# TheNeodev/RVC-MAKER

Measured on AMD Instinct MI355X. Metric: audio-seconds/sec/GPU (xRT) end-to-end VC, 48k v2; 1/2/4/8 GPU scaling, higher is better.
Workload: dtype f32-equivalent (split-fp16 3-pass MFMA for the generator's convs -- scale from the producer's published |max| -- and ResBlock pairs, split-bf16 6-pass MFMA elsewhere; f32 accumulate; RMVPE f64 with its GRU recurrence f32); 1 GPU; VC.pipeline 48k v2, ContentVec-768, rmvpe f0, one 30 s clip per GPU per step, no index, protect 0.33, clip stream (clip k+1 f0/features under clip k synthesizer); model=RVC v2 48k (NSF-HiFiGAN) + ContentVec + rmvpe, global_batch=1, seq_len=480000, parallelism=utterance-sharded x1

## Files before the change

### include/rvc_amd.h

```cpp
#ifndef RVC_AMD_H
#define RVC_AMD_H

#include <stdint.h>

#ifdef __cplusplus
extern "C" {
#endif

typedef struct ihipStream_t* rvc_stream_t;

enum { RVC_OK = 0, RVC_EINVAL = -22, RVC_EHIP = -5 };

enum {
    RVC_ACT_NONE = 0,
    RVC_ACT_LRELU = 1,
    RVC_ACT_RELU = 2,
    RVC_ACT_TANH = 3,
    RVC_ACT_GELU = 4,
    RVC_ACT_SIGMOID = 5,
    RVC_ACT_LOGCLAMP = 6,
};

const char* rvc_last_error(void);
int rvc_version(void);
// ... 20 lines not shown
    int toff[16];
    const void* wx;
    int wx_nmf, wx_passes;
    const unsigned* amax_in;
    unsigned* amax_out;
    const float* src_x;
    const float* src_w;
    const float* src_b;
    int src_K, src_stride, src_pad, _pad1;
    int64_t src_len, src_bstride;
} rvc_conv1d_args;

int64_t rvc_conv1d_workspace_bytes(const rvc_conv1d_args* a);
int rvc_conv1d_engine(const rvc_conv1d_args* a);
int rvc_conv1d_tile(const rvc_conv1d_args* a);
int rvc_conv1d(const rvc_conv1d_args* a, void* ws, int64_t ws_bytes, rvc_stream_t stream);
void rvc_conv1d_set_probe_event(void* hip_event);
int rvc_conv1d_set_stamps(void* buf, int64_t bytes);
int rvc_resblock_set_stamps(void* buf, int64_t bytes);
int rvc_resblock_set_ylds(int on);
int rvc_resblock_set_wide64(int on);
int rvc_conv1d_set_tile_epi(int on);
int rvc_conv1d_set_swz(int on);
int rvc_conv1d_set_f16_fast(int on);
int rvc_conv1d_set_splitk_target(int target);
int rvc_stream_create_cu_mask(const uint32_t* mask, int nwords, rvc_stream_t* out);
int rvc_stream_destroy(rvc_stream_t stream);
int64_t rvc_conv1d_x6_bytes(int64_t nphase, int64_t Ci, int K, int64_t Co);
int rvc_conv1d_pack_x6(const float* w_km, int64_t nphase, int64_t Ci, int K, int64_t Co, void* out, int* nmf_out,
                       rvc_stream_t stream);
int64_t rvc_conv1d_f16_bytes(int64_t nphase, int64_t Ci, int K, int64_t Co);
int rvc_conv1d_pack_f16(const float* w_km, int64_t nphase, int64_t Ci, int K, int64_t Co, void* out, int* nmf_out,
                        rvc_stream_t stream);

typedef struct rvc_resblock_args {
    const float* x;
    float* y;
    const void* w1x;
    const float* b1;
    const void* w2x;
    const float* b2;
    int64_t C, L;
    int K, dil, nmf1, nmf2, passes, accumulate;
    float slope;
    int B;
} rvc_resblock_args;
// ... 456 lines not shown
```

### rvc-maker_amd/csrc/conv1d.hip

```cpp
#include "rvc_common.h"
#include "x6_common.h"
#include <stdlib.h>
#include <type_traits>
#include <algorithm>

namespace {

constexpr int KCH = 32;
constexpr int NB_MAX = 16;

struct ConvParams {
    const float* x;
    const float* w;
    const float* bias;
    const float* bias2;
    const float* res;
    float* y;
    float* ws;
    int64_t B, Ci, Co, Lin, Lout, ncols;
    int64_t x_bstride, y_bstride, res_bstride, w_bstride;
    int K, stride, dil, pad, groups;
    int nphase, ostride, ooffset;
    int in_act, out_act, accumulate;
    float in_scale, in_slope, out_slope, out_scale;
    int span, span_s, rows_max;
    float inv_span;
    int mtiles_per_group, ksplit, chunks_per_split, avec;
    int ntoff, wrap;
    int toff[16];
    const uint4* wx;
    int wx_nmf, wx_nch, wx_passes;
    int rot;
    int xcd;
    int dbg;
    int tile_epi;
    const unsigned* amax_in;
    int f16_fast;
    unsigned* amax_out;
    int stagger;
    int stagger_blocks;
    int swz;
    int gx6;
#if RVC_CONV_STAMPS
    unsigned long long* stamps;
    int64_t stamp_blocks;
#endif
};

static thread_local int g_f16_fast = -1;
static thread_local int g_swz = -1;

__device__ __forceinline__ int tap_off(const ConvParams& p, int t) { return p.ntoff ? p.toff[t] : t * p.dil; }

__device__ __forceinline__ int out_pos(const ConvParams& p, int64_t n, int phase) {
    if (n >= p.ncols) return -1;
    const int t = (int)n * p.ostride + p.ooffset + phase;
    if (t < 0 || t >= (int)p.Lout) return -1;
    if (p.wrap) {
        const int row = t / p.wrap, col = t - row * p.wrap;
        if (col == 0 || col == p.wrap - 1 || row == 0 || row == (int)p.Lout / p.wrap - 1) return -(t + 2);
    }
    return t;
}

__device__ __forceinline__ float epilogue_store(const ConvParams& p, float acc, int b, int64_t m, int t) {
    const bool ok = t >= 0;
    const int64_t o = m * p.Lout + (ok ? t : 0);
    float v = acc;
    if (p.bias) v += p.bias[m];
    if (p.bias2) v += p.bias2[m];
    v = act_apply(v, p.out_act, p.out_slope) * p.out_scale;
    if (p.res) v += p.res[b * p.res_bstride + o];
    float* yb = p.y + b * p.y_bstride;
// ... 648 lines not shown
    }
    if (p.amax_out && !part) amax_publish(p.amax_out + (int64_t)b * RVC_AMAX_SHARDS, amx);
}

template <int FM, int FN, int WM, int WN, int X6_NI, int NP, bool F16, bool SA = false, int LF = 0>
__global__ __launch_bounds__(64 * (WM * WN + 4), (x6_min_blocks<FM, FN, WM * WN, NP>())) void conv_x6_kernel(ConvParams p) {
    static_assert(WM * WN == 4 || WM * WN == 8, "4 or 8 compute waves");
    constexpr int NCW = WM * WN;
    static_assert(NP == 6 || NP == 3 || NP == 1, "6, 3 or 1 passes");
    static_assert(!F16 || NP == 3, "split-fp16: 3 passes");
    static_assert(!SA || (NP == 6 && !F16), "split accumulators: 6-pass split-bf16");
    static_assert(LF == 0 || (F16 && WM * WN == 8), "fast-only loaders: split-fp16 on 8 compute waves");
    constexpr int NPL = NP == 6 ? 3 : (NP == 3 ? 2 : 1);
    constexpr int BM = 16 * FM * WM;
    constexpr int BN = 16 * FN * WN;
    extern __shared__ uint4 xs[];
    const int tid = threadIdx.x, lane = tid & 63;
    const int wave = __builtin_amdgcn_readfirstlane(tid >> 6);
    int bx = blockIdx.x, by = blockIdx.y, bz = blockIdx.z;
    if (p.xcd) {
        const int nx = gridDim.x, ny = gridDim.y;
        const int nwg = nx * ny * (int)gridDim.z;
        const int orig = bx + nx * (by + ny * bz);
        const int q = nwg >> 3, r = nwg & 7, xc = orig & 7;
        const int t = (xc < r ? xc * (q + 1) : r * (q + 1) + (xc - r) * q) + (orig >> 3);
        bx = t % nx;
        by = (t / nx) % ny;
        bz = t / (nx * ny);
    }
    int zb = bz;
    const int split = zb % p.ksplit;
    zb /= p.ksplit;
    const int phase = zb % p.nphase;
    const int b = zb / p.nphase;
    const int grp = p.gx6 ? phase : 0;
    const int ophase = p.gx6 ? 0 : phase;
    const int Cog = (int)p.Co;
    const int Cig = (int)p.Ci;
    const int m0g = by * BM;
    const int64_t n0 = (int64_t)bx * BN;
    const int K = p.K, span = p.span;
    const int nch = p.wx_nch, nmf = p.wx_nmf;
    const int ch_beg = split * p.chunks_per_split;
    const int ch_end = min(nch, ch_beg + p.chunks_per_split);
    const int nck = ch_end - ch_beg;
    const int bufsz = NPL * span * 4;
    float* tmax = reinterpret_cast<float*>(xs + 2 * bufsz);
    float* etab = tmax + 4;
    const int rseed = p.rot ? (bx >> 3) : 0;
    const int rt = rseed % K, rc = (rseed / K) % max(nck, 1);
    auto pchunk = [&](int i) __attribute__((always_inline)) {
// ... 567 lines not shown
        }
    }
    float yo[SRC_M];
#pragma unroll
    for (int mi = 0; mi < SRC_M; ++mi) yo[mi] = yb[(int64_t)(m0 + (mi < nm ? mi : 0)) * p.Lout];
    float amx = 0.f;
#pragma unroll
    for (int mi = 0; mi < SRC_M; ++mi) {
        if (mi < nm) {
            const int m = m0 + mi;
            const float v = (acc[mi] + (p.b ? p.b[m] : 0.f)) + yo[mi];
            if (ok) {
                yb[(int64_t)m * p.Lout] = v;
                amx = fmaxf(amx, fabsf(v));
            }
        }
    }
    if (p.amax_out) amax_publish_block(p.amax_out + (int64_t)b * RVC_AMAX_SHARDS, amx);
}

struct Cfg {
    int FM, FN, WM, WN;
    bool x6;
};

template <int FM, int FN, int WM, int WN>
hipError_t launch(const ConvParams& p, dim3 grid, size_t lds, hipStream_t s) {
    hipLaunchKernelGGL((conv1d_mfma_kernel<FM, FN, WM, WN>), grid, dim3(256), lds, s, p);
    return hipGetLastError();
}

template <int FM, int FN, int WM, int WN, int NP, bool F16 = false, bool SA = false, int LF = 0>
void launch_x6_np(const ConvParams& p, dim3 grid, size_t lds, hipStream_t s) {
    const dim3 blk(64 * (WM * WN + 4));
    if (4 * p.span <= 256 * 3)
        hipLaunchKernelGGL((conv_x6_kernel<FM, FN, WM, WN, 3, NP, F16, SA, LF>), grid, blk, lds, s, p);
    else hipLaunchKernelGGL((conv_x6_kernel<FM, FN, WM, WN, 6, NP, F16, SA, LF>), grid, blk, lds, s, p);
}

int x6_f16_fast_form(const ConvParams& p) {
    if (!p.amax_in || !p.f16_fast || (p.Ci & 31) != 0 || p.in_scale != 1.f) return 0;
    return p.in_act == RVC_ACT_LRELU ? 1 : (p.in_act == RVC_ACT_NONE ? 2 : 0);
}

constexpr bool x6_sa_tile(int FM, int FN, int WM, int WN) {
    return (WM * WN == 8 && FN == 4) || (WM * WN == 4 && FM <= 2 && FN == 2) || (WM == 2 && WN == 4);
// ... 39 lines not shown
    for (int i = 0; i < 16; ++i) p.toff[i] = a->ntoff ? a->toff[i] : 0;
    p.wx = nullptr;
    p.wx_nmf = p.wx_nch = 0;
    p.wx_passes = a->wx_passes == 0 ? 6 : a->wx_passes;
    static const int dbg = getenv("RVC_CONV_DEBUG") ? atoi(getenv("RVC_CONV_DEBUG")) : 0;
    p.dbg = dbg;
    p.tile_epi = 0;
    p.amax_in = a->amax_in;
    p.amax_out = a->amax_out;
    static const int f16fast = getenv("RVC_X6_F16FAST") ? atoi(getenv("RVC_X6_F16FAST")) : 1;
    p.f16_fast = g_f16_fast >= 0 ? g_f16_fast : f16fast;
    p.stagger = 0;
    p.stagger_blocks = 0;
    static const int swz_env = getenv("RVC_X6_SWZ") ? atoi(getenv("RVC_X6_SWZ")) : 1;
    p.swz = g_swz >= 0 ? g_swz : swz_env;
    p.gx6 = 0;
#if RVC_CONV_STAMPS
    p.stamps = g_stamps;
    p.stamp_blocks = g_stamp_blocks;
#endif
    static const int rot = getenv("RVC_X6_ROT") ? atoi(getenv("RVC_X6_ROT")) : 0;
    p.rot = rot;
    static const int xcd = getenv("RVC_X6_XCD") ? atoi(getenv("RVC_X6_XCD")) : 1;
    p.xcd = xcd;
}

int num_cus() {
    static const int n = [] {
        int dev = 0, cus = 0;
        if (hipGetDevice(&dev) != hipSuccess ||
            hipDeviceGetAttribute(&cus, hipDeviceAttributeMultiprocessorCount, dev) != hipSuccess || cus <= 0)
            cus = 256;
        return cus;
    }();
    return n;
}

static thread_local int g_splitk_target = -1;
static thread_local int g_tile_epi = -1;

void split_k(ConvParams& p, int64_t tiles, int nch, int per_cu = 2) {
    static const int env_target = getenv("RVC_SPLITK_TILES") ? atoi(getenv("RVC_SPLITK_TILES")) : 256;
    static const int occ_aware = getenv("RVC_X6_SPLIT_OCC") ? atoi(getenv("RVC_X6_SPLIT_OCC")) : 1;
    int target = g_splitk_target >= 0 ? g_splitk_target : env_target;
    if (occ_aware && per_cu == 1 && g_splitk_target < 0) target /= 2;
    int ks = 1;
    if (tiles < target && nch >= 4) {
// ... 38 lines not shown

int plan(const rvc_conv1d_args* a, ConvParams& p, Cfg& cfg, dim3& grid, size_t& lds) {
    RVC_CHECK_ARG(a && a->x && a->w && a->y, "conv1d: null pointer");
    RVC_CHECK_ARG(a->B > 0 && a->Ci > 0 && a->Co > 0 && a->K > 0 && a->Lin > 0 && a->Lout > 0,
                  "conv1d: bad sizes B=%lld Ci=%lld Co=%lld K=%d Lin=%lld Lout=%lld", (long long)a->B,
                  (long long)a->Ci, (long long)a->Co, a->K, (long long)a->Lin, (long long)a->Lout);
    RVC_CHECK_ARG(a->groups >= 1 && a->Ci % a->groups == 0 && a->Co % a->groups == 0, "conv1d: bad groups");
    RVC_CHECK_ARG(a->stride >= 1 && a->dil >= 1 && a->nphase >= 1 && a->ostride >= 1, "conv1d: bad stride/dil");
    RVC_CHECK_ARG(a->Co * a->Lout < (1ll << 31) && a->Ci * a->Lin < (1ll << 31) && a->Lin + a->pad < (1ll << 30),
                  "conv1d: per-batch tensor exceeds 2^31 elements (use the batch dimension)");
    const int64_t Cog = a->Co / a->groups;
    const int64_t Cig = a->Ci / a->groups;
    const int64_t ncols = a->ncols > 0 ? a->ncols : a->Lout;
    fill_common(a, p);
    RVC_CHECK_ARG(!a->src_x || (a->src_w && a->src_K > 0 && a->src_K <= 4096 && a->src_stride > 0 && a->src_pad >= 0 &&
                                a->src_len > 0 && a->src_bstride >= 0 && !a->wrap),
                  "conv1d: bad fused source conv (src_K=%d src_stride=%d src_pad=%d src_len=%lld)", a->src_K,
                  a->src_stride, a->src_pad, (long long)a->src_len);
    RVC_CHECK_ARG(!a->src_x || ((int64_t)255 * a->src_stride + 17 * a->src_K) * 4 <= 64 * 1024,
                  "conv1d: source conv span too large (stride %d, K %d)", a->src_stride, a->src_K);
    if (a->ntoff) {
        RVC_CHECK_ARG(a->ntoff == a->K && a->K <= 16, "conv1d: toff needs ntoff == K <= 16");
        for (int i = 0; i < a->K; ++i) RVC_CHECK_ARG(a->toff[i] >= 0, "conv1d: negative tap offset");
    }

    if (x6_eligible(a)) {
        cfg.x6 = true;
        static const int w8 = getenv("RVC_X6_W8") ? atoi(getenv("RVC_X6_W8")) : 1;
        const int np = a->wx_passes == 0 || a->wx_passes == RVC_ARITH_FP32_SA ? 6 : a->wx_passes;
        static const int bn256 = getenv("RVC_X6_BN256") ? atoi(getenv("RVC_X6_BN256")) : 1;
        auto round_eff = [](int64_t t) {
            const int64_t n = num_cus();
            return (double)t / (double)(((t + n - 1) / n) * n);
        };
        const int64_t rows128 = (Cog + 127) / 128, nb = a->B * a->nphase;
        const bool fills256 = round_eff(rows128 * ((ncols + 255) / 256) * nb) >=
                              round_eff(rows128 * ((ncols + 127) / 128) * nb) - 0.05;
        if (Cog > 64 && w8 && bn256 && a->stride == 1 && 255 + max_tap_off(a) + 1 <= 64 * X6_NI_MAX - 2 &&
            Cog % 16 == 0 && a->Lout < (1ll << 26) && ncols < (1ll << 26) &&
            (bn256 == 2 || np == RVC_ARITH_F16X3) && (fills256 || bn256 == 3))
            cfg = {2, 8, 4, 2, true};
        else if (Cog > 64 && w8) cfg = {2, 4, 4, 2, true};
        else if (Cog > 64) cfg = {4, 4, 2, 2, true};
        else if (Cog > 32 && w8 && np >= 3) cfg = {2, 2, 2, 4, true};
        else if (Cog > 32) cfg = {2, 4, 2, 2, true};
        else if (Cog > 16) cfg = {2, 2, 1, 4, true};
// ... 1 lines not shown
        RVC_CHECK_ARG(a->wx_passes != RVC_ARITH_FP32_SA || x6_sa_tile(cfg.FM, cfg.FN, cfg.WM, cfg.WN),
                      "conv1d: RVC_ARITH_FP32_SA has no split-accumulator kernel for the %dx%d tile on %d waves "
                      "(engine switches changed?)", 16 * cfg.FM * cfg.WM, 16 * cfg.FN * cfg.WN, cfg.WM * cfg.WN);
        const int BM = 16 * cfg.FM * cfg.WM, BN = 16 * cfg.FN * cfg.WN;
        p.span = (BN - 1) * a->stride + max_tap_off(a) + 1;
        p.span_s = p.span;
        p.rows_max = 0;
        p.inv_span = 1.0f / (float)p.span;
        p.avec = 0;
        p.wx = (const uint4*)a->wx;
        p.wx_nmf = a->wx_nmf;
        p.wx_nch = (int)((Cig + 31) / 32);
        p.mtiles_per_group = (int)((Cog + BM - 1) / BM);
        const int64_t tiles = (int64_t)p.mtiles_per_group * ((ncols + BN - 1) / BN) * a->B * a->nphase * a->groups;
        split_k(p, tiles, p.wx_nch, cfg.WM * cfg.WN == 8 ? 1 : 2);
        if (a->groups > 1) {
            p.gx6 = 1;
            p.nphase = a->groups;
            p.Ci = Cig;
            p.Co = Cog;
            p.chunks_per_split = p.wx_nch;
            p.ksplit = 1;
        }
        lds = (size_t)2 * (p.wx_passes == 6 || p.wx_passes == RVC_ARITH_FP32_SA ? 3 : (p.wx_passes == 1 ? 1 : 2)) *
              p.span * 64 + 16;
        static const int tepi_env = getenv("RVC_X6_TILE_EPI") ? atoi(getenv("RVC_X6_TILE_EPI")) : 0;
        const int tepi = g_tile_epi >= 0 ? g_tile_epi : tepi_env;
        const size_t tile_bytes = (size_t)BM * (BN + 4) * 4;
        const bool plain = a->nphase == 1 && a->ostride == 1 && a->ooffset == 0 && !a->wrap && !(p.dbg & 1) &&
                           BN <= 128;
        p.tile_epi = !(tepi && plain && a->groups == 1) ? 0
                     : tile_bytes <= lds ? 1 : (cfg.WM % 2 == 0 && tile_bytes / 2 <= lds) ? 2 : 0;
        lds += (size_t)3 * BM * 4;
        grid = dim3(cdiv(ncols, BN), (unsigned)p.mtiles_per_group, (unsigned)(a->B * p.nphase * p.ksplit));
        RVC_CHECK_ARG(grid.y < 65536 && grid.z < 65536, "conv1d: grid too large");
        static const int stagger = getenv("RVC_X6_STAGGER") ? atoi(getenv("RVC_X6_STAGGER")) : 0;
        static const int stagger_rounds = getenv("RVC_X6_STAGGER_ROUNDS") ? atoi(getenv("RVC_X6_STAGGER_ROUNDS")) : 2;
        const int64_t nblk = (int64_t)grid.x * grid.y * grid.z;
        if (stagger > 0 && nblk >= stagger_rounds * (int64_t)num_cus()) {
            p.stagger = stagger;
            p.stagger_blocks = num_cus();
        }
        return RVC_OK;
    }

    if (Cog % 48 == 0 && Cog % 64 != 0) cfg = {3, 1, 1, 4, false};
// ... 139 lines not shown
    RVC_CHECK_ARG(w_km && out && nmf_out && nphase > 0 && Ci > 0 && K > 0 && Co > 0, "pack_f16: bad args");
    const int nch = (int)((Ci + 31) / 32), nmf = (int)x6_nmf(Co);
    const int64_t total = nphase * K * nch * nmf * 3 * 64;
    float* rs = reinterpret_cast<float*>(reinterpret_cast<uint4*>(out) + total);
    hipStream_t s = (hipStream_t)stream;
    const int64_t nrow = nphase * Ci * K;
    RVC_HIP(hipMemsetAsync(rs, 0, (size_t)nmf * 16 * 4, s));
    hipLaunchKernelGGL(rowscale_f16_kernel, dim3(cdiv(Co, 64), (unsigned)std::min<int64_t>(64, cdiv(nrow, 64))),
                       dim3(256), 0, s, w_km, nrow, (int)Co, reinterpret_cast<unsigned*>(rs));
    hipLaunchKernelGGL(rowscale_fin_kernel, dim3(cdiv(nmf * 16, 256)), dim3(256), 0, s, rs, nmf * 16);
    hipLaunchKernelGGL(pack_f16_kernel, dim3(cdiv(total, 256)), dim3(256), 0, s, w_km, total, (int)Ci, K, (int)Co, nch,
                       nmf, (const float*)rs, (uint4*)out);
    RVC_HIP(hipGetLastError());
    *nmf_out = nmf;
    return RVC_OK;
}

extern "C" int rvc_conv1d_engine(const rvc_conv1d_args* a) {
    ConvParams p;
    Cfg cfg;
    dim3 grid;
    size_t lds;
    if (plan(a, p, cfg, grid, lds) != RVC_OK) return -1;
    return cfg.x6 ? 1 : 0;
}

extern "C" int rvc_conv1d_tile(const rvc_conv1d_args* a) {
    ConvParams p;
    Cfg cfg;
    dim3 grid;
    size_t lds;
    if (plan(a, p, cfg, grid, lds) != RVC_OK) return -1;
    return (16 * cfg.FM * cfg.WM) << 16 | (16 * cfg.FN * cfg.WN);
}

extern "C" int64_t rvc_conv1d_workspace_bytes(const rvc_conv1d_args* a) {
    ConvParams p;
    Cfg cfg;
    dim3 grid;
    size_t lds;
    if (plan(a, p, cfg, grid, lds) != RVC_OK) return -1;
    if (p.ksplit <= 1) return 0;
    return (int64_t)p.ksplit * p.B * p.nphase * p.Co * p.ncols * 4;
}

extern "C" int rvc_conv1d_set_splitk_target(int target) {
    const int prev = g_splitk_target;
    g_splitk_target = target < 0 ? -1 : target;
    return prev;
}

static thread_local hipEvent_t g_probe_event = nullptr;

extern "C" void rvc_conv1d_set_probe_event(void* hip_event) { g_probe_event = (hipEvent_t)hip_event; }

extern "C" int rvc_conv1d_set_f16_fast(int on) {
    g_f16_fast = on < 0 ? -1 : (on ? 1 : 0);
    return RVC_OK;
}

extern "C" int rvc_conv1d_set_swz(int on) {
    g_swz = on < 0 ? -1 : (on ? 1 : 0);
    return RVC_OK;
}

extern "C" int rvc_conv1d_set_tile_epi(int on) {
    g_tile_epi = on < 0 ? -1 : (on ? 1 : 0);
    return RVC_OK;
}

extern "C" int rvc_conv1d_set_stamps(void* buf, int64_t bytes) {
#if RVC_CONV_STAMPS
    g_stamps = (unsigned long long*)buf;
    g_stamp_blocks = buf ? bytes / (8 * X6_STAMP_W) : 0;
    return 0;
#else
    (void)buf;
    (void)bytes;
    return -1;
#endif
}

extern "C" int rvc_conv1d(const rvc_conv1d_args* a, void* ws, int64_t ws_bytes, rvc_stream_t stream) {
    ConvParams p;
    Cfg cfg;
    dim3 grid;
    size_t lds;
    int rc = plan(a, p, cfg, grid, lds);
    if (rc != RVC_OK) return rc;
    if (p.ksplit > 1) {
        const int64_t need = (int64_t)p.ksplit * p.B * p.nphase * p.Co * p.ncols * 4;
        RVC_CHECK_ARG(ws && ws_bytes >= need, "conv1d: split-K needs %lld B of workspace (got %lld)",
                      (long long)need, (long long)ws_bytes);
        p.ws = (float*)ws;
    }
    hipStream_t s = (hipStream_t)stream;
    if (a->src_x) p.amax_out = nullptr;
    hipError_t e;
    if (cfg.x6) {
        if (cfg.WM == 4 && cfg.FN == 8) e = launch_x6<2, 8, 4, 2>(p, grid, lds, s);
        else if (cfg.WM == 4) e = launch_x6<2, 4, 4, 2>(p, grid, lds, s);
        else if (cfg.WM == 2 && cfg.WN == 4) e = launch_x6<2, 2, 2, 4>(p, grid, lds, s);
        else if (cfg.FM == 4) e = launch_x6<4, 4, 2, 2>(p, grid, lds, s);
        else if (cfg.WM == 2) e = launch_x6<2, 4, 2, 2>(p, grid, lds, s);
        else if (cfg.FM == 2) e = launch_x6<2, 2, 1, 4>(p, grid, lds, s);
        else e = launch_x6<1, 2, 1, 4>(p, grid, lds, s);
    } else if (cfg.FM == 3) e = launch<3, 1, 1, 4>(p, grid, lds, s);
    else if (cfg.FM == 1 && cfg.FN == 4) e = launch<1, 4, 1, 4>(p, grid, lds, s);
    else if (cfg.FM == 1) e = launch<1, 2, 1, 4>(p, grid, lds, s);
    else if (cfg.WM == 1 && cfg.FN == 4) e = launch<2, 4, 1, 4>(p, grid, lds, s);
    else if (cfg.WM == 1) e = launch<2, 2, 1, 4>(p, grid, lds, s);
    else if (cfg.FM == 4 && cfg.FN == 4) e = launch<4, 4, 2, 2>(p, grid, lds, s);
    else if (cfg.FM == 4) e = launch<4, 2, 2, 2>(p, grid, lds, s);
    else if (cfg.FN == 4) e = launch<2, 4, 2, 2>(p, grid, lds, s);
    else e = launch<2, 2, 2, 2>(p, grid, lds, s);
    RVC_HIP(e);
    if (g_probe_event) RVC_HIP(hipEventRecord(g_probe_event, s));
    if (p.ksplit > 1) {
        hipLaunchKernelGGL(conv_splitk_reduce,
// ... 27 lines not shown
```

### rvc-maker_amd/csrc/model_common.h

```cpp
#pragma once
#include <hip/hip_runtime_api.h>
#include <math.h>
#include <stdint.h>
#include <stdlib.h>
#include <string.h>

#include <map>
#include <string>
#include <vector>

#include "../../include/rvc_amd.h"

void rvc_set_error(const char* fmt, ...);

#define MCHECK(cond, ...)               \
    do {                                \
        if (!(cond)) {                  \
            rvc_set_error(__VA_ARGS__); \
            return RVC_EINVAL;          \
        }                               \
    } while (0)
#define MHIP(call)                                                  \
    do {                                                            \
        hipError_t e_ = (call);                                     \
// ... 1 lines not shown
            rvc_set_error("%s: %s", #call, hipGetErrorString(e_)); \
            return RVC_EHIP;                                        \
        }                                                           \
    } while (0)
#define MTRY(call)                     \
    do {                               \
        int rc_ = (call);              \
        if (rc_ != RVC_OK) return rc_; \
    } while (0)

struct Synth;
struct ContentVec;
struct Rmvpe;
struct Crepe;
struct VcState;

struct rvc_ctx {
    int device = 0;
    int prec = RVC_PREC_FP32;
    int rm_prec = RVC_PREC_FP64;
    bool x6 = true, f16mix = true, fused_rb = true;
    bool amax = true;
    bool amax_f16all = true;
    bool cv_amax = true;
    bool amax_ups = true;
    bool amax_s2 = true;
    bool fe_amax = true;
    bool fused_noise = false;
    bool attn_f16 = true;
    bool te_amax = false;
    bool flow_amax = false;
    Synth* syn = nullptr;
    ContentVec* cv = nullptr;
    Rmvpe* rm = nullptr;
    Crepe* cr = nullptr;
    VcState* vc = nullptr;
};

void synth_delete(Synth* s);
void contentvec_delete(ContentVec* m);
void rmvpe_delete(Rmvpe* m);
void crepe_delete(Crepe* m);
void vc_delete(VcState* v);

int synth_run_cf(rvc_ctx* c, const float* phone_cf, const int64_t* pitch, const float* pitchf, int64_t T, int64_t sid,
                 uint64_t seed, float* wav, hipStream_t s);
// ... 193 lines not shown
    cw.Co = w.dim(1);
    cw.Kfull = (int)w.dim(2);
    cw.u = u;
    cw.tpad = pad;
    cw.nphase = u;
    const int T = (cw.Kfull + u - 1) / u;
    cw.K = T;
    std::vector<float> km((size_t)u * cw.Ci * T * cw.Co, 0.f);
    for (int r = 0; r < u; ++r)
        for (int tp = 0; tp < T; ++tp) {
            const int j = r + (T - 1 - tp) * u;
            if (j >= cw.Kfull) continue;
            for (int64_t ci = 0; ci < cw.Ci; ++ci)
                for (int64_t mo = 0; mo < cw.Co; ++mo)
                    km[(((int64_t)r * cw.Ci + ci) * T + tp) * cw.Co + mo] = w.v[(ci * cw.Co + mo) * cw.Kfull + j];
        }
    MTRY(upload(m, km, &cw.w));
    MTRY(upload(m, b.v, &cw.b));
    return make_images(c, m, cw);
}

inline int base_passes(const rvc_ctx* c) { return c->prec == RVC_PREC_FP32 ? 6 : c->prec; }

inline int conv_passes(const rvc_ctx* c, int K, int64_t Cig, int stride, bool two_d, bool amax = false) {
    if (c->prec == RVC_PREC_FP32 && c->f16mix && !two_d &&
        ((stride == 1 && ((amax && c->amax_f16all) || (K >= 7 && Cig <= 256) || (K >= 3 && Cig >= 64 && Cig <= 128))) ||
         (stride == 2 && amax && c->amax_f16all && c->amax_s2)))
        return RVC_ARITH_F16X3;
    return base_passes(c);
}

inline int ensure_ws(ModelBase& m, int64_t need, hipStream_t s) {
    if (need <= m.ws_bytes) return RVC_OK;
    if (m.ws) {
        MHIP(hipStreamSynchronize(s));
        MHIP(hipFree(m.ws));
        m.ws = nullptr;
        m.ws_bytes = 0;
    }
    const int64_t bytes = need + (4 << 20);
    MHIP(hipMalloc(&m.ws, bytes));
    m.ws_bytes = bytes;
    return RVC_OK;
}

inline int ensure_arena(ModelBase& m, int64_t floats, hipStream_t s) {
    if (floats <= m.arena_floats) return RVC_OK;
// ... 68 lines not shown
        a.src_bstride = o.src_len;
    }
    int stride = o.stride;
    if (cw.nphase > 1) {
        const int64_t Lout = (Lin - 1) * cw.u - 2 * cw.tpad + cw.Kfull;
        a.Lout = Lout;
        a.ncols = (Lout - 1 + cw.tpad) / cw.u + 1;
        a.stride = 1;
        a.pad = cw.K - 1;
        a.dil = 1;
        a.nphase = cw.u;
        a.ostride = cw.u;
        a.ooffset = -cw.tpad;
        stride = 1;
    } else {
        a.Lout = o.Lout >= 0 ? o.Lout : (Lin + 2 * o.pad - o.dil * (cw.K - 1) - 1) / o.stride + 1;
        a.stride = o.stride;
        a.pad = o.pad;
        a.dil = o.dil;
        a.nphase = 1;
        a.ostride = 1;
    }
    if (cw.wx_bf) {
        const int passes = conv_passes(c, cw.K, cw.Ci / cw.groups, stride, o.ntoff > 0, o.amax_in != nullptr);
        a.wx = passes == RVC_ARITH_F16X3 ? cw.wx_hf : cw.wx_bf;
        a.wx_nmf = cw.nmf;
        a.wx_passes = passes;
    }
    const int64_t need = rvc_conv1d_workspace_bytes(&a);
    if (need < 0) return RVC_EINVAL;
    MTRY(ensure_ws(m, need, s));
    return rvc_conv1d(&a, need ? m.ws : nullptr, need, s);
}

struct Scratch {
    float* base = nullptr;
    int64_t off = 0;
    bool dry = true;
    float* take(int64_t n) {
        float* p = dry ? (float*)(uintptr_t)(256 + off * 4) : base + off;
        off += (n + 63) & ~int64_t(63);
        return p;
    }
};
#define RUN(call)              \
    do {                       \
        if (!sc.dry) MTRY(call); \
// ... 23 lines not shown
```

### rvc-maker_amd/csrc/rvc_model.cpp

```cpp
#include "model_common.h"

using namespace rvcm;

namespace synthm {

constexpr float kLreluSlope = 0.1f;

struct Pair {
    int d;
    ConvW c1, c2;
};

struct Layer {
    ConvW qkv, relk, o, ffn1, ffn2;
    float *ev = nullptr, *ln1g = nullptr, *ln1b = nullptr, *ln2g = nullptr, *ln2b = nullptr;
};

struct Flow {
    ConvW pre, post;
    ConvW ins[3], rs_a[2], rs_b[3];
};

}

// ... 383 lines not shown
    op.in_act = RVC_ACT_LRELU;
    op.in_slope = 0.01f;
    op.in_scale = scale_in;
    op.out_act = RVC_ACT_TANH;
    return conv(c, S, S.conv_post, xcur, Lcur, wav, op, s);
}

}

using namespace synthm;


extern "C" int rvc_ctx_create(int hip_device, rvc_ctx** out) {
    MCHECK(out, "rvc_ctx_create: null out");
    *out = nullptr;
    MHIP(hipSetDevice(hip_device));
    rvc_ctx* c = new rvc_ctx();
    c->device = hip_device;
    c->x6 = env_on("RVC_AMD_X6");
    c->f16mix = env_on("RVC_AMD_F16MIX");
    c->fused_rb = env_on("RVC_AMD_FUSED_RB");
    c->amax = env_on("RVC_AMD_AMAX");
    c->amax_f16all = env_on("RVC_AMD_AMAX_F16ALL");
    c->cv_amax = env_on("RVC_AMD_CV_AMAX");
    c->amax_ups = env_on("RVC_AMD_AMAX_UPS");
    c->amax_s2 = env_on("RVC_AMD_AMAX_S2");
    c->fe_amax = env_on("RVC_AMD_FE_AMAX");
    c->fused_noise = env_set("RVC_AMD_FUSED_NOISE");
    c->attn_f16 = env_on("RVC_AMD_ATTN_F16");
    c->te_amax = env_set("RVC_AMD_TE_AMAX");
    c->flow_amax = env_set("RVC_AMD_FLOW_AMAX");
    *out = c;
    return RVC_OK;
}

extern "C" void rvc_ctx_destroy(rvc_ctx* c) {
    if (!c) return;
    if (hipSetDevice(c->device) == hipSuccess) {
        (void)hipDeviceSynchronize();
        synth_delete(c->syn);
        vc_delete(c->vc);
        contentvec_delete(c->cv);
        rmvpe_delete(c->rm);
        crepe_delete(c->cr);
    }
    delete c;
// ... 279 lines not shown
```

### rvc-maker_amd/rvc_amd/_lib.py

```python
from __future__ import annotations

import ctypes
import os
from ctypes import POINTER, c_double, c_float, c_int, c_int64, c_uint64, c_void_p

LIB_PATH = os.environ.get("RVC_AMD_LIB") or os.path.join(
    os.path.dirname(os.path.dirname(os.path.abspath(__file__))), "lib", "librvc_amd.so")

ACT_NONE, ACT_LRELU, ACT_RELU, ACT_TANH, ACT_GELU, ACT_SIGMOID, ACT_LOGCLAMP = 0, 1, 2, 3, 4, 5, 6
LFILTER_CHUNK, LFILTER_WAVE, LFILTER_TILE, LFILTER_WARM_CAP = 512, 64 * 512, 32, 16384


class Conv1dArgs(ctypes.Structure):
    _fields_ = [("x", c_void_p), ("w", c_void_p), ("bias", c_void_p), ("bias2", c_void_p), ("res", c_void_p),
                ("y", c_void_p),
                ("B", c_int64), ("Ci", c_int64), ("Co", c_int64), ("Lin", c_int64), ("Lout", c_int64),
                ("ncols", c_int64), ("x_bstride", c_int64), ("y_bstride", c_int64), ("res_bstride", c_int64),
                ("w_bstride", c_int64),
                ("K", c_int), ("stride", c_int), ("dil", c_int), ("pad", c_int), ("groups", c_int),
                ("nphase", c_int), ("ostride", c_int), ("ooffset", c_int),
                ("in_act", c_int), ("out_act", c_int), ("accumulate", c_int), ("_pad0", c_int),
                ("in_scale", c_float), ("in_slope", c_float), ("out_slope", c_float), ("out_scale", c_float),
                ("ntoff", c_int), ("wrap", c_int), ("toff", c_int * 16),
                ("wx", c_void_p), ("wx_nmf", c_int), ("wx_passes", c_int),
# ... 82 lines not shown
    _fields_ = [("f0_method", c_int), ("f0_autotune", c_int), ("f0_autotune_strength", c_double),
                ("f0_file", c_void_p), ("f0_file_rows", c_int64), ("volume_envelope", c_double),
                ("crepe_dither", c_void_p)]


class IvfIndex(ctypes.Structure):
    _fields_ = [("d", c_int64), ("nlist", c_int64), ("ntotal", c_int64), ("nprobe", c_int), ("_pad0", c_int),
                ("centroids", c_void_p), ("list_off", c_void_p), ("codes", c_void_p), ("ids", c_void_p),
                ("big", c_void_p)]


SIGNATURES = {
    "rvc_last_error": [],
    "rvc_version": [],
    "rvc_conv1d": [POINTER(Conv1dArgs), c_void_p, c_int64, c_void_p],
    "rvc_conv1d_workspace_bytes": [POINTER(Conv1dArgs)],
    "rvc_conv1d_set_probe_event": [c_void_p],
    "rvc_conv1d_set_stamps": [c_void_p, c_int64],
    "rvc_resblock_set_stamps": [c_void_p, c_int64],
    "rvc_resblock_set_ylds": [c_int],
    "rvc_resblock_set_wide64": [c_int],
    "rvc_conv1d_set_tile_epi": [c_int],
    "rvc_conv1d_set_swz": [c_int],
    "rvc_conv1d_set_f16_fast": [c_int],
    "rvc_bigru64_set_f32": [c_int],
    "rvc_conv1d_set_splitk_target": [c_int],
    "rvc_stream_create_cu_mask": [c_void_p, c_int, POINTER(c_void_p)],
    "rvc_stream_destroy": [c_void_p],
    "rvc_conv1d_engine": [POINTER(Conv1dArgs)],
    "rvc_conv1d_tile": [POINTER(Conv1dArgs)],
    "rvc_conv1d_x6_bytes": [c_int64, c_int64, c_int, c_int64],
    "rvc_conv1d_pack_x6": [c_void_p, c_int64, c_int64, c_int, c_int64, c_void_p, POINTER(c_int), c_void_p],
    "rvc_conv1d_f16_bytes": [c_int64, c_int64, c_int, c_int64],
    "rvc_pm_frames": [c_int64],
    "rvc_pm_work_bytes": [c_int64],
    "rvc_pm_f0": [c_void_p, c_int64, c_void_p, c_void_p, c_void_p, c_int64, c_void_p, c_void_p],
    "rvc_pm_post": [c_void_p, c_int64, c_int64, ctypes.c_double, c_void_p, c_void_p, c_void_p, c_void_p],
    "rvc_swipe_frames": [c_int64],
    "rvc_swipe_work_bytes": [c_int64],
    "rvc_swipe_tables_bytes": [],
    "rvc_swipe_table_dims": [c_int, c_int, POINTER(c_int64)],
    "rvc_swipe_tables": [c_void_p, c_int64],
    "rvc_swipe_strength": [c_void_p, c_int64, c_void_p, c_void_p, c_int64, c_void_p, c_void_p],
    "rvc_swipe_pick": [c_void_p, c_int64, c_void_p, c_void_p, c_void_p],
    "rvc_swipe_post": [c_void_p, c_int64, c_float, POINTER(F0Post), c_void_p, c_void_p, c_void_p],
    "rvc_abs_quantile_work_bytes": [],
    "rvc_abs_quantile": [c_void_p, c_int64, c_void_p, c_int64, c_void_p, c_void_p],
    "rvc_abs_quantile_as": [c_void_p, c_int64, c_int, c_void_p, c_int64, c_void_p, c_void_p],
    "rvc_div_scalar": [c_void_p, c_int64, c_void_p, c_void_p, c_void_p],
    "rvc_f0_mix": [POINTER(F0Track), c_int, c_int64, c_void_p, c_void_p],
    "rvc_f0_resample_nan": [c_void_p, c_int64, c_int64, c_void_p, c_void_p],
    "rvc_fcpe_mel": [c_void_p, c_void_p, c_void_p, c_int64, c_int64, c_void_p],
    "rvc_groupnorm_work_bytes": [c_int64, c_int],
# ... 228 lines not shown
```

### rvc-maker_amd/rvc_amd/ops.py

```python
from __future__ import annotations

import ctypes
import math
import os

import numpy as np
import torch

from . import _lib
from ._lib import ACT_GELU, ACT_LOGCLAMP, ACT_LRELU, ACT_NONE, ACT_RELU, ACT_SIGMOID, ACT_TANH, check


def _stream():
    return ctypes.c_void_p(torch.cuda.current_stream().cuda_stream)


def _p(t):
    if t is None:
        return None
    if not t.is_cuda or t.dtype not in (torch.float32, torch.int64, torch.int32, torch.uint8):
        raise TypeError(f"rvc_amd: expected a CUDA f32/int tensor, got {t.dtype} on {t.device}")
    return ctypes.c_void_p(t.data_ptr())


# ... 5 lines not shown

def pack_convT(w: torch.Tensor, u: int) -> tuple[torch.Tensor, int]:
    Ci, Co, K = w.shape
    T = -(-K // u)
    out = torch.zeros(u, Ci, T, Co, dtype=w.dtype)
    for r in range(u):
        for tp in range(T):
            j = r + (T - 1 - tp) * u
            if j < K:
                out[r, :, tp, :] = w[:, :, j]
    return out.reshape(u, Ci * T, Co).contiguous(), T


X6 = os.environ.get("RVC_AMD_X6", "1") != "0"

F16X3 = 16
PASSES = {"fp32": 6, "fp32x6": 6, "fp32sa": 7, "f16x3": F16X3, "bf16x3": 3, "bf16": 1}
F16_MIX = os.environ.get("RVC_AMD_F16MIX", "1") != "0"
AMAX_F16ALL = os.environ.get("RVC_AMD_AMAX_F16ALL", "1") != "0"
AMAX_SHARDS = 64
AMAX_S2 = os.environ.get("RVC_AMD_AMAX_S2", "1") != "0"


def conv_passes(K, Ci, stride=1, two_d=False, amax=False):
    if _PRECISION == "fp32" and F16_MIX and not two_d and \
            ((stride == 1 and ((amax and AMAX_F16ALL) or (K >= 7 and Ci <= 256) or (K >= 3 and 64 <= Ci <= 128))) or
             (stride == 2 and amax and AMAX_F16ALL and AMAX_S2)):
        return F16X3
    return PASSES[_PRECISION]
_PRECISION = os.environ.get("RVC_AMD_PRECISION", "fp32")
if _PRECISION not in PASSES:
    raise ValueError(f"RVC_AMD_PRECISION must be one of {sorted(PASSES)}")


def get_precision() -> str:
    return _PRECISION


def set_precision(name: str) -> str:
    global _PRECISION
    if name not in PASSES:
        raise ValueError(f"precision must be one of {sorted(PASSES)}, got {name!r}")
    prev, _PRECISION = _PRECISION, name
    return prev


class splitk_target:
# ... 208 lines not shown
    a.in_scale, a.in_slope, a.out_slope, a.out_scale = in_scale, in_slope, out_slope, out_scale
    if toff is not None:
        if len(toff) != K or K > 16:
            raise ValueError("conv1d: toff must have K <= 16 entries")
        a.ntoff = K
        for i, v in enumerate(toff):
            a.toff[i] = int(v)
    a.wrap = wrap
    a.amax_in, a.amax_out = _p(amax_in), _p(amax_out)
    for cell in (amax_in, amax_out):
        if cell is not None and cell.numel() < B * AMAX_SHARDS:
            raise ValueError(f"conv1d: a |max| cell needs {AMAX_SHARDS} words per batch element (B={B})")
    if src is not None:
        sconv, sig, s_stride, s_pad = src
        if sconv.Ci != 1 or sconv.groups != 1 or sconv.Co != Co:
            raise ValueError("conv1d: src needs a 1-input-channel conv with the output's channels")
        s_len = sig.shape[-1]
        if sig.dim() not in (1, 2) or (sig.dim() == 2 and sig.shape[0] != B) or not sig.is_contiguous() or \
                (sig.dim() == 1 and B != 1):
            raise ValueError("conv1d: src signal must be contiguous [B][N]")
        a.src_x, a.src_w, a.src_b = _p(sig), _p(sconv.w), _p(sconv.b)
        a.src_K, a.src_stride, a.src_pad, a.src_len, a.src_bstride = sconv.K, s_stride, s_pad, s_len, s_len
    if wx is not None:
        passes = conv_passes(K, Ci // groups, stride, toff is not None, amax_in is not None)
        a.wx, a.wx_nmf, a.wx_passes = ctypes.c_void_p(wx.data_ptr(passes)), wx_nmf, passes
    if flops is None:
        valid = (Lout // wrap - 2) * (wrap - 2) if wrap else (ncols or Lout) * nphase
        flops = 2.0 * B * Co * Cig * K * min(valid, Lout)
    LAST_CONV_FLOPS = flops
    lib = _lib.load()
    need = lib.rvc_conv1d_workspace_bytes(ctypes.byref(a))
    if need < 0:
        raise RuntimeError(f"rvc_amd: conv1d plan failed: {lib.rvc_last_error().decode()}")
    ws = _workspace(out.device, need) if need else None
    LAST_CONV_WS = need
    LAST_CONV_ENGINE = lib.rvc_conv1d_engine(ctypes.byref(a))
    LAST_CONV_PASSES = a.wx_passes if LAST_CONV_ENGINE == 1 else 0
    _LAST_CONV_ARGS = a
    check(lib.rvc_conv1d(ctypes.byref(a), _p(ws), need, _stream()), "conv1d")
    return out


FUSED_RB = os.environ.get("RVC_AMD_FUSED_RB", "1") != "0"
RB_PASSES = (6, 3, 1, F16X3)


RB_F16_KMIN = int(os.environ.get("RVC_AMD_RB_F16_KMIN", "3"))
# ... 964 lines not shown
```

Before: 1192 audio-s/s.

## Add direct f32 skinny-conv kernel for Co<=4 and phase-major x6 block ordering

```diff
diff --git a/include/rvc_amd.h b/include/rvc_amd.h
--- a/include/rvc_amd.h
+++ b/include/rvc_amd.h
@@ -66,6 +66,9 @@
 int rvc_resblock_set_wide64(int on);
 int rvc_conv1d_set_tile_epi(int on);
 int rvc_conv1d_set_swz(int on);
+int rvc_conv1d_set_phase_order(int on);
+int rvc_conv1d_set_direct(int on);
+int rvc_conv1d_phase_order(const rvc_conv1d_args* a);
 int rvc_conv1d_set_f16_fast(int on);
 int rvc_conv1d_set_splitk_target(int target);
 int rvc_stream_create_cu_mask(const uint32_t* mask, int nwords, rvc_stream_t* out);
diff --git a/rvc-maker_amd/csrc/conv1d.hip b/rvc-maker_amd/csrc/conv1d.hip
--- a/rvc-maker_amd/csrc/conv1d.hip
+++ b/rvc-maker_amd/csrc/conv1d.hip
@@ -3,6 +3,10 @@
 #include <stdlib.h>
 #include <type_traits>
 #include <algorithm>
+
+bool rvc_skinny_conv_eligible(const rvc_conv1d_args* a);
+int rvc_skinny_conv_tile(const rvc_conv1d_args* a);
+int rvc_skinny_conv_launch(const rvc_conv1d_args* a, hipStream_t s);
 
 namespace {
 
@@ -49,6 +53,8 @@
 
 static thread_local int g_f16_fast = -1;
 static thread_local int g_swz = -1;
+static thread_local int g_phase_order = -1;
+static thread_local int g_direct = -1;
 
 __device__ __forceinline__ int tap_off(const ConvParams& p, int t) { return p.ntoff ? p.toff[t] : t * p.dil; }
 
@@ -743,11 +749,24 @@
         const int nx = gridDim.x, ny = gridDim.y;
         const int nwg = nx * ny * (int)gridDim.z;
         const int orig = bx + nx * (by + ny * bz);
-        const int q = nwg >> 3, r = nwg & 7, xc = orig & 7;
-        const int t = (xc < r ? xc * (q + 1) : r * (q + 1) + (xc - r) * q) + (orig >> 3);
-        bx = t % nx;
-        by = (t / nx) % ny;
-        bz = t / (nx * ny);
+        int t = orig;
+        if (p.xcd & 1) {
+            const int q = nwg >> 3, r = nwg & 7, xc = orig & 7;
+            t = (xc < r ? xc * (q + 1) : r * (q + 1) + (xc - r) * q) + (orig >> 3);
+        }
+        if (p.xcd & 2) {
+            const int ph = t % p.nphase;
+            int r = t / p.nphase;
+            bx = r % nx;
+            r /= nx;
+            by = r % ny;
+            r /= ny;
+            bz = r % p.ksplit + p.ksplit * (ph + p.nphase * (r / p.ksplit));
+        } else {
+            bx = t % nx;
+            by = (t / nx) % ny;
+            bz = t / (nx * ny);
+        }
     }
     int zb = bz;
     const int split = zb % p.ksplit;
@@ -1361,6 +1380,7 @@
 struct Cfg {
     int FM, FN, WM, WN;
     bool x6;
+    bool direct = false;
 };
 
 template <int FM, int FN, int WM, int WN>
@@ -1446,7 +1466,7 @@
     static const int rot = getenv("RVC_X6_ROT") ? atoi(getenv("RVC_X6_ROT")) : 0;
     p.rot = rot;
     static const int xcd = getenv("RVC_X6_XCD") ? atoi(getenv("RVC_X6_XCD")) : 1;
-    p.xcd = xcd;
+    p.xcd = xcd ? 1 : 0;
 }
 
 int num_cus() {
@@ -1531,6 +1551,17 @@
     if (a->ntoff) {
         RVC_CHECK_ARG(a->ntoff == a->K && a->K <= 16, "conv1d: toff needs ntoff == K <= 16");
         for (int i = 0; i < a->K; ++i) RVC_CHECK_ARG(a->toff[i] >= 0, "conv1d: negative tap offset");
+    }
+
+    static const int direct_env = getenv("RVC_CONV_DIRECT") ? atoi(getenv("RVC_CONV_DIRECT")) : 1;
+    if ((g_direct >= 0 ? g_direct : direct_env) && rvc_skinny_conv_eligible(a)) {
+        cfg = {0, 0, 0, 0, false};
+        cfg.direct = true;
+        p.ksplit = 1;
+        p.chunks_per_split = 0;
+        grid = dim3(1);
+        lds = 0;
+        return RVC_OK;
     }
 
     if (x6_eligible(a)) {
@@ -1578,6 +1609,8 @@
             p.chunks_per_split = p.wx_nch;
             p.ksplit = 1;
         }
+        static const int phord_env = getenv("RVC_X6_PHASE_ORDER") ? atoi(getenv("RVC_X6_PHASE_ORDER")) : 1;
+        if ((g_phase_order >= 0 ? g_phase_order : phord_env) && p.nphase > 1 && !p.gx6) p.xcd |= 2;
         lds = (size_t)2 * (p.wx_passes == 6 || p.wx_passes == RVC_ARITH_FP32_SA ? 3 : (p.wx_passes == 1 ? 1 : 2)) *
               p.span * 64 + 16;
         static const int tepi_env = getenv("RVC_X6_TILE_EPI") ? atoi(getenv("RVC_X6_TILE_EPI")) : 0;
@@ -1763,7 +1796,7 @@
     dim3 grid;
     size_t lds;
     if (plan(a, p, cfg, grid, lds) != RVC_OK) return -1;
-    return cfg.x6 ? 1 : 0;
+    return cfg.direct ? 3 : (cfg.x6 ? 1 : 0);
 }
 
 extern "C" int rvc_conv1d_tile(const rvc_conv1d_args* a) {
@@ -1772,7 +1805,17 @@
     dim3 grid;
     size_t lds;
     if (plan(a, p, cfg, grid, lds) != RVC_OK) return -1;
+    if (cfg.direct) return rvc_skinny_conv_tile(a);
     return (16 * cfg.FM * cfg.WM) << 16 | (16 * cfg.FN * cfg.WN);
+}
+
+extern "C" int rvc_conv1d_phase_order(const rvc_conv1d_args* a) {
+    ConvParams p;
+    Cfg cfg;
+    dim3 grid;
+    size_t lds;
+    if (plan(a, p, cfg, grid, lds) != RVC_OK) return -1;
+    return cfg.x6 ? (p.xcd >> 1) & 1 : 0;
 }
 
 extern "C" int64_t rvc_conv1d_workspace_bytes(const rvc_conv1d_args* a) {
@@ -1802,6 +1845,16 @@
 
 extern "C" int rvc_conv1d_set_swz(int on) {
     g_swz = on < 0 ? -1 : (on ? 1 : 0);
+    return RVC_OK;
+}
+
+extern "C" int rvc_conv1d_set_phase_order(int on) {
+    g_phase_order = on < 0 ? -1 : (on ? 1 : 0);
+    return RVC_OK;
+}
+
+extern "C" int rvc_conv1d_set_direct(int on) {
+    g_direct = on < 0 ? -1 : (on ? 1 : 0);
     return RVC_OK;
 }
 
@@ -1836,6 +1889,12 @@
         p.ws = (float*)ws;
     }
     hipStream_t s = (hipStream_t)stream;
+    if (cfg.direct) {
+        rc = rvc_skinny_conv_launch(a, s);
+        if (rc != RVC_OK) return rc;
+        if (g_probe_event) RVC_HIP(hipEventRecord(g_probe_event, s));
+        return RVC_OK;
+    }
     if (a->src_x) p.amax_out = nullptr;
     hipError_t e;
     if (cfg.x6) {
diff --git a/rvc-maker_amd/csrc/model_common.h b/rvc-maker_amd/csrc/model_common.h
--- a/rvc-maker_amd/csrc/model_common.h
+++ b/rvc-maker_amd/csrc/model_common.h
@@ -47,6 +47,7 @@
     bool x6 = true, f16mix = true, fused_rb = true;
     bool amax = true;
     bool amax_f16all = true;
+    bool conv_direct = true;
     bool cv_amax = true;
     bool amax_ups = true;
     bool amax_s2 = true;
@@ -286,7 +287,10 @@
 
 inline int base_passes(const rvc_ctx* c) { return c->prec == RVC_PREC_FP32 ? 6 : c->prec; }
 
-inline int conv_passes(const rvc_ctx* c, int K, int64_t Cig, int stride, bool two_d, bool amax = false) {
+inline int conv_passes(const rvc_ctx* c, int K, int64_t Cig, int stride, bool two_d, bool amax = false, int64_t Co = 0) {
+    if (c->prec == RVC_PREC_FP32 && c->conv_direct && Co > 0 && Co <= 4 && stride == 1 && !two_d &&
+        (K == 3 || K == 5 || K == 7))
+        return 6;
     if (c->prec == RVC_PREC_FP32 && c->f16mix && !two_d &&
         ((stride == 1 && ((amax && c->amax_f16all) || (K >= 7 && Cig <= 256) || (K >= 3 && Cig >= 64 && Cig <= 128))) ||
          (stride == 2 && amax && c->amax_f16all && c->amax_s2)))
@@ -401,7 +405,8 @@
         a.ostride = 1;
     }
     if (cw.wx_bf) {
-        const int passes = conv_passes(c, cw.K, cw.Ci / cw.groups, stride, o.ntoff > 0, o.amax_in != nullptr);
+        const int passes = conv_passes(c, cw.K, cw.Ci / cw.groups, stride, o.ntoff > 0, o.amax_in != nullptr,
+                                       cw.nphase > 1 || cw.groups > 1 ? 0 : cw.Co);
         a.wx = passes == RVC_ARITH_F16X3 ? cw.wx_hf : cw.wx_bf;
         a.wx_nmf = cw.nmf;
         a.wx_passes = passes;
diff --git a/rvc-maker_amd/csrc/rvc_model.cpp b/rvc-maker_amd/csrc/rvc_model.cpp
--- a/rvc-maker_amd/csrc/rvc_model.cpp
+++ b/rvc-maker_amd/csrc/rvc_model.cpp
@@ -429,6 +429,7 @@
     c->fused_rb = env_on("RVC_AMD_FUSED_RB");
     c->amax = env_on("RVC_AMD_AMAX");
     c->amax_f16all = env_on("RVC_AMD_AMAX_F16ALL");
+    c->conv_direct = env_on("RVC_CONV_DIRECT");
     c->cv_amax = env_on("RVC_AMD_CV_AMAX");
     c->amax_ups = env_on("RVC_AMD_AMAX_UPS");
     c->amax_s2 = env_on("RVC_AMD_AMAX_S2");
diff --git a/rvc-maker_amd/csrc/skinny.hip b/rvc-maker_amd/csrc/skinny.hip
--- /dev/null
+++ b/rvc-maker_amd/csrc/skinny.hip
@@ -0,0 +1,189 @@
+#include "rvc_common.h"
+#include <stdlib.h>
+
+namespace {
+
+constexpr int SK_NT = 256;
+constexpr int SK_ROW = 4 * SK_NT;
+constexpr int SK_TW = 252;
+constexpr int SK_T = 4 * SK_TW;
+constexpr int SK_CC = 8;
+constexpr int SK_KMAX = 9;
+static_assert(4 * (SK_TW - 1) + 3 + SK_KMAX - 1 + 3 < SK_ROW, "the last window, shifted by the alignment slack, is staged");
+
+struct SkinnyParams {
+    const float* x;
+    const float* w;
+    const float* bias;
+    float* y;
+    unsigned* amax_out;
+    int64_t x_bstride, y_bstride;
+    int Ci, Co, Lin, Lout, pad;
+    int in_act, out_act;
+    float in_scale, in_slope, out_slope, out_scale;
+    int xvec, yvec;
+};
+
+template <int K, int CO>
+__global__ __launch_bounds__(SK_NT) void conv_skinny_kernel(SkinnyParams p) {
+    static_assert(K <= SK_KMAX && CO <= 4, "window / accumulator budget");
+    __shared__ __attribute__((aligned(16))) float sx[SK_CC][SK_ROW + 4];
+    const int tid = threadIdx.x, b = blockIdx.y;
+    const int t0 = blockIdx.x * SK_T;
+    const int q0 = t0 - p.pad;
+    const int a0 = q0 & ~3;
+    const int off = q0 - a0;
+    const int qv = a0 + 4 * tid;
+    const int Lin = p.Lin, Ci = p.Ci;
+    const float* xb = p.x + (int64_t)b * p.x_bstride;
+    const bool vec = p.xvec && qv >= 0 && qv + 3 < Lin;
+    const bool any = qv + 3 >= 0 && qv < Lin;
+
+    float4 r[SK_CC];
+    auto load = [&](int c0) __attribute__((always_inline)) {
+        if (vec) {
+#pragma unroll
+            for (int i = 0; i < SK_CC; ++i) {
+                const int c = c0 + i < Ci ? c0 + i : Ci - 1;
+                r[i] = *reinterpret_cast<const float4*>(xb + (int64_t)c * Lin + qv);
+            }
+        } else if (any) {
+#pragma unroll
+            for (int i = 0; i < SK_CC; ++i) {
+                const int c = c0 + i < Ci ? c0 + i : Ci - 1;
+                const float* row = xb + (int64_t)c * Lin;
+                float e[4];
+#pragma unroll
+                for (int j = 0; j < 4; ++j) {
+                    const int q = qv + j;
+                    const float v = row[q < 0 ? 0 : (q >= Lin ? Lin - 1 : q)];
+                    e[j] = (q >= 0 && q < Lin) ? v : 0.f;
+                }
+                r[i] = make_float4(e[0], e[1], e[2], e[3]);
+            }
+        } else {
+#pragma unroll
+            for (int i = 0; i < SK_CC; ++i) r[i] = make_float4(0.f, 0.f, 0.f, 0.f);
+        }
+    };
+    auto pre = [&](float v) __attribute__((always_inline)) {
+        v *= p.in_scale;
+        if (p.in_act == RVC_ACT_LRELU) v = v >= 0.f ? v : v * p.in_slope;
+        return v;
+    };
+    auto stage = [&](int c0) __attribute__((always_inline)) {
+        const int j0 = 4 * tid - off;
+#pragma unroll
+        for (int i = 0; i < SK_CC; ++i) {
+            const bool cin = c0 + i < Ci;
+            const float4 v = make_float4(cin ? pre(r[i].x) : 0.f, cin ? pre(r[i].y) : 0.f, cin ? pre(r[i].z) : 0.f,
+                                         cin ? pre(r[i].w) : 0.f);
+            if (off == 0) {
+                *reinterpret_cast<float4*>(&sx[i][j0]) = v;
+            } else {
+                if (j0 >= 0) sx[i][j0] = v.x;
+                if (j0 + 1 >= 0) sx[i][j0 + 1] = v.y;
+                if (j0 + 2 >= 0) sx[i][j0 + 2] = v.z;
+                sx[i][j0 + 3] = v.w;
+            }
+        }
+    };
+
+    float acc[CO][4];
+#pragma unroll
+    for (int m = 0; m < CO; ++m)
+#pragma unroll
+        for (int j = 0; j < 4; ++j) acc[m][j] = 0.f;
+
+    load(0);
+    for (int c0 = 0; c0 < Ci; c0 += SK_CC) {
+        stage(c0);
+        __syncthreads();
+        if (c0 + SK_CC < Ci) load(c0 + SK_CC);
+        if (tid < SK_TW) {
+            const int nc = Ci - c0 < SK_CC ? Ci - c0 : SK_CC;
+            for (int i = 0; i < nc; ++i) {
+                float win[12];
+#pragma unroll
+                for (int q = 0; q < 3; ++q) {
+                    const float4 v = *reinterpret_cast<const float4*>(&sx[i][4 * tid + 4 * q]);
+                    win[4 * q] = v.x, win[4 * q + 1] = v.y, win[4 * q + 2] = v.z, win[4 * q + 3] = v.w;
+                }
+                const float* wc = p.w + (int64_t)(c0 + i) * K * p.Co;
+#pragma unroll
+                for (int k = 0; k < K; ++k)
+#pragma unroll
+                    for (int m = 0; m < CO; ++m) {
+                        const float wv = m < p.Co ? wc[k * p.Co + m] : 0.f;
+#pragma unroll
+                        for (int j = 0; j < 4; ++j) acc[m][j] = fmaf(wv, win[j + k], acc[m][j]);
+                    }
+            }
+        }
+        __syncthreads();
+    }
+
+    const int t = t0 + 4 * tid;
+    float* yb = p.y + (int64_t)b * p.y_bstride;
+    float amx = 0.f;
+#pragma unroll
+    for (int m = 0; m < CO; ++m) {
+        if (m < p.Co && tid < SK_TW) {
+            float bs = 0.f;
+            if (p.bias) bs = p.bias[m];
+            float v[4];
+#pragma unroll
+            for (int j = 0; j < 4; ++j) v[j] = act_apply(acc[m][j] + bs, p.out_act, p.out_slope) * p.out_scale;
+            float* row = yb + (int64_t)m * p.Lout;
+            if (p.yvec && t + 3 < p.Lout) {
+                *reinterpret_cast<float4*>(row + t) = make_float4(v[0], v[1], v[2], v[3]);
+#pragma unroll
+                for (int j = 0; j < 4; ++j) amx = fmaxf(amx, fabsf(v[j]));
+            } else {
+#pragma unroll
+                for (int j = 0; j < 4; ++j)
+                    if (t + j < p.Lout) {
+                        row[t + j] = v[j];
+                        amx = fmaxf(amx, fabsf(v[j]));
+                    }
+            }
+        }
+    }
+    if (p.amax_out) amax_publish_block(p.amax_out + (int64_t)b * RVC_AMAX_SHARDS, amx);
+}
+
+template <int K>
+void launch_skinny(const SkinnyParams& p, dim3 grid, hipStream_t s) {
+    if (p.Co == 1) hipLaunchKernelGGL((conv_skinny_kernel<K, 1>), grid, dim3(SK_NT), 0, s, p);
+    else hipLaunchKernelGGL((conv_skinny_kernel<K, 4>), grid, dim3(SK_NT), 0, s, p);
+}
+
+}
+
+bool rvc_skinny_conv_eligible(const rvc_conv1d_args* a) {
+    return a->groups == 1 && a->Co <= 4 && (a->K == 3 || a->K == 5 || a->K == 7) && a->stride == 1 && a->dil == 1 &&
+           a->nphase == 1 && a->ostride == 1 && a->ooffset == 0 && (a->ncols == 0 || a->ncols == a->Lout) && !a->wrap &&
+           !a->ntoff && !a->w_bstride && !a->src_x && !a->bias2 && !a->res && !a->accumulate &&
+           (a->in_act == RVC_ACT_NONE || a->in_act == RVC_ACT_LRELU) && (a->wx_passes == 0 || a->wx_passes == 6) &&
+           a->pad >= 0 && a->Lin < (1ll << 30) && a->Lout < (1ll << 30) && a->B < 65536;
+}
+
+int rvc_skinny_conv_tile(const rvc_conv1d_args* a) { return ((a->Co == 1 ? 1 : 4) << 16) | SK_T; }
+
+int rvc_skinny_conv_launch(const rvc_conv1d_args* a, hipStream_t s) {
+    SkinnyParams p;
+    p.x = a->x; p.w = a->w; p.bias = a->bias; p.y = a->y; p.amax_out = a->amax_out;
+    p.x_bstride = a->x_bstride ? a->x_bstride : a->Ci * a->Lin;
+    p.y_bstride = a->y_bstride ? a->y_bstride : a->Co * a->Lout;
+    p.Ci = (int)a->Ci; p.Co = (int)a->Co; p.Lin = (int)a->Lin; p.Lout = (int)a->Lout; p.pad = a->pad;
+    p.in_act = a->in_act; p.out_act = a->out_act;
+    p.in_scale = a->in_scale; p.in_slope = a->in_slope; p.out_slope = a->out_slope; p.out_scale = a->out_scale;
+    p.xvec = a->Lin % 4 == 0 && ((uintptr_t)a->x & 15) == 0 && p.x_bstride % 4 == 0;
+    p.yvec = a->Lout % 4 == 0 && ((uintptr_t)a->y & 15) == 0 && p.y_bstride % 4 == 0;
+    const dim3 grid(cdiv(a->Lout, SK_T), (unsigned)a->B);
+    if (a->K == 3) launch_skinny<3>(p, grid, s);
+    else if (a->K == 5) launch_skinny<5>(p, grid, s);
+    else launch_skinny<7>(p, grid, s);
+    RVC_HIP(hipGetLastError());
+    return RVC_OK;
+}
diff --git a/rvc-maker_amd/rvc_amd/_lib.py b/rvc-maker_amd/rvc_amd/_lib.py
--- a/rvc-maker_amd/rvc_amd/_lib.py
+++ b/rvc-maker_amd/rvc_amd/_lib.py
@@ -128,6 +128,8 @@
     "rvc_resblock_set_wide64": [c_int],
     "rvc_conv1d_set_tile_epi": [c_int],
     "rvc_conv1d_set_swz": [c_int],
+    "rvc_conv1d_set_phase_order": [c_int],
+    "rvc_conv1d_set_direct": [c_int],
     "rvc_conv1d_set_f16_fast": [c_int],
     "rvc_bigru64_set_f32": [c_int],
     "rvc_conv1d_set_splitk_target": [c_int],
@@ -135,6 +137,7 @@
     "rvc_stream_destroy": [c_void_p],
     "rvc_conv1d_engine": [POINTER(Conv1dArgs)],
     "rvc_conv1d_tile": [POINTER(Conv1dArgs)],
+    "rvc_conv1d_phase_order": [POINTER(Conv1dArgs)],
     "rvc_conv1d_x6_bytes": [c_int64, c_int64, c_int, c_int64],
     "rvc_conv1d_pack_x6": [c_void_p, c_int64, c_int64, c_int, c_int64, c_void_p, POINTER(c_int), c_void_p],
     "rvc_conv1d_f16_bytes": [c_int64, c_int64, c_int, c_int64],
diff --git a/rvc-maker_amd/rvc_amd/ops.py b/rvc-maker_amd/rvc_amd/ops.py
--- a/rvc-maker_amd/rvc_amd/ops.py
+++ b/rvc-maker_amd/rvc_amd/ops.py
@@ -51,7 +51,13 @@
 AMAX_S2 = os.environ.get("RVC_AMD_AMAX_S2", "1") != "0"
 
 
-def conv_passes(K, Ci, stride=1, two_d=False, amax=False):
+CONV_DIRECT = os.environ.get("RVC_CONV_DIRECT", "1") != "0"
+
+
+def conv_passes(K, Ci, stride=1, two_d=False, amax=False, Co=None):
+    if _PRECISION == "fp32" and CONV_DIRECT and Co is not None and Co <= 4 and stride == 1 and not two_d and \
+            K in (3, 5, 7):
+        return PASSES["fp32"]
     if _PRECISION == "fp32" and F16_MIX and not two_d and \
             ((stride == 1 and ((amax and AMAX_F16ALL) or (K >= 7 and Ci <= 256) or (K >= 3 and 64 <= Ci <= 128))) or
              (stride == 2 and amax and AMAX_F16ALL and AMAX_S2)):
@@ -306,7 +312,8 @@
         a.src_x, a.src_w, a.src_b = _p(sig), _p(sconv.w), _p(sconv.b)
         a.src_K, a.src_stride, a.src_pad, a.src_len, a.src_bstride = sconv.K, s_stride, s_pad, s_len, s_len
     if wx is not None:
-        passes = conv_passes(K, Ci // groups, stride, toff is not None, amax_in is not None)
+        passes = conv_passes(K, Ci // groups, stride, toff is not None, amax_in is not None,
+                             Co if groups == 1 and nphase == 1 else None)
         a.wx, a.wx_nmf, a.wx_passes = ctypes.c_void_p(wx.data_ptr(passes)), wx_nmf, passes
     if flops is None:
         valid = (Lout // wrap - 2) * (wrap - 2) if wrap else (ncols or Lout) * nphase
```

New measurement: 1192 audio-s/s. No clear change (-0.0%).
